# gvanhorn38/multibox

Measured on AMD Instinct MI355X. Metric: images/sec (299x299, 5-AR priors) train, higher is better.
Workload: dtype bf16; 1 GPU; full train step: Inception-ResNet-v2 + multibox heads fwd, on-device matching+loss, bwd, RMSProp+EMA; 299x299, k=5 (P=646), BATCH_SIZE=64/GPU, MAX_NUM_BBOXES=13; global_batch=64, parallelism=dp1, hip_graph=True

## Files before the change

include/mbx.h:

```cpp
#ifndef MBX_H
#define MBX_H

#include <stddef.h>
#include <stdint.h>

#ifdef __cplusplus
extern "C" {
#endif

typedef void* mbx_stream_t;

typedef enum {
  MBX_OK = 0,
  MBX_ERR_INVALID_ARG = -1,
  MBX_ERR_UNSUPPORTED = -2,
  MBX_ERR_LAUNCH = -3,
  MBX_ERR_WORKSPACE = -4
} mbx_status;

int mbx_version(void);
const char* mbx_status_string(int status);

int mbx_priors_count(int k, const int* grids, int n_grids);

// ... 96 lines not shown
                   int32_t* n_gt_counted , int32_t* status , mbx_stream_t stream);

#define MBX_COCO_ACC_MAX_R 128
#define MBX_COCO_ACC_MAX_M 4
#define MBX_COCO_ACC_MAX_ND 4194304
#define MBX_COCO_ACC_CHUNK 256
#define MBX_COCO_ACC_SORT_TILE 1024
size_t mbx_coco_accumulate_workspace(long long ND, int T, int A, int M);
int mbx_coco_accumulate(const double* dt , const int32_t* dt_rows , int I,
                        const int16_t* match , const uint8_t* ignore ,
                        const int32_t* n_gt_counted , int T, int A, const double* rec_thrs , int R,
                        const int32_t* max_dets , int M, double* precision ,
                        double* recall , void* workspace, size_t workspace_bytes, mbx_stream_t stream);

typedef enum {
  MBX_EPI_STORE = 0,
  MBX_EPI_AFFINE = 1,
  MBX_EPI_RESIDUAL = 2,
  MBX_EPI_STORE_F32 = 3
} mbx_epilogue;

typedef struct {
  int32_t n, rows_mod;
  int32_t c_begin[4];
  const void* y[4]; int32_t ld_y[4];
  const float* relu_thr[4];
  float* stats[4]; int32_t stats_ld[4];
} mbx_bn_bwd_stats;

#define MBX_GRID_BARRIER_BYTES 6400
typedef struct {
  void* barrier;
  void* a; int32_t ld_a;
  const float* beta;
  float* mean; float* rstd;
  float* moving_mean; float* moving_var;
  float* relu_thr;
  int32_t relu; float eps, decay;
  float* step_poison;
} mbx_bn_apply_desc;

#define MBX_BN_BWD_SLOTS 8
typedef struct {
  void* barrier;
  int32_t n;
  int32_t c_begin[4];
  const void* y[4]; int32_t ld_y[4];
  void* dy[4]; int32_t ld_dy[4];
  const float* mean[4]; const float* rstd[4]; const float* beta[4];
  float* dbeta[4];
  float* acc[4]; int32_t acc_ld[4];
  int32_t relu[4];
  float* step_poison;
} mbx_bn_bwd_fused;

typedef struct {
  const void* x; int64_t x_img_stride; int32_t ldx;
  int32_t N, H_in, W_in, C_in;
  const void* w; int32_t C_out, R, S;
  int32_t stride, transposed, pad_t, pad_l, H_out, W_out;
  void* y; int64_t y_img_stride; int32_t ldy;
  int32_t epilogue, relu, accumulate;
  const float* scale; const float* shift;
  const void* skip; int64_t skip_img_stride; int32_t ld_skip; float rscale;
  float* stats_partial;
  int32_t tile_config;
  const void* acc_src; int64_t acc_img_stride; int32_t ld_acc;
  int32_t* work_counter;
  int32_t max_workgroups;
  void* splitk_ws; int64_t splitk_ws_bytes;
  int32_t stats_rows_mod, stats_ld;
  const mbx_bn_bwd_stats* bn_bwd_stats;
  void* relu_bits; int32_t ld_bits;
  const mbx_bn_apply_desc* bn_apply;
  const mbx_bn_bwd_fused* bn_bwd;
} mbx_conv_desc;
#define MBX_CONV_TILE_CONFIGS 14
#define MBX_TILE_I5_BASE 32
#define MBX_TILE_I7 65
#define MBX_TILE_DIRECT3 96
#define MBX_TILE_DIRECTW 97
#define MBX_TILE_RESIDENT 98
#define MBX_TILE_PWRES 99
#define MBX_TILE_SPLITK_BASE 128
#define MBX_TILE_SPLITK_MAX 32

int mbx_conv_stats_rows(const mbx_conv_desc* desc );
int mbx_conv(const mbx_conv_desc* desc , mbx_stream_t stream);
int mbx_conv_supported(const mbx_conv_desc* desc );
int mbx_conv_pair(const mbx_conv_desc* a , const mbx_conv_desc* b , mbx_stream_t stream);
size_t mbx_conv_splitk_workspace_bytes(const mbx_conv_desc* desc );

int mbx_conv_wgrad(const mbx_conv_desc* desc , const void* dy,
                   int64_t dy_img_stride, int32_t ld_dy, float* dw, float* db, mbx_stream_t stream);

typedef struct {
  mbx_conv_desc desc;
  const void* dy; int64_t dy_img_stride; int32_t ld_dy;
  float scale;
  float* dw; float* db;
} mbx_wgrad_job;
typedef struct {
  int32_t n_layers, n_items;
  int64_t layers_off, items_off;
  int64_t queues_off, heads_off;
  double flops;
  int64_t tally_off;
} mbx_wgrad_plan_info;
#define MBX_WGRAD_DETERMINISTIC 1
#define MBX_WGRAD_SCATTER 2
size_t mbx_wgrad_plan_bytes(const mbx_wgrad_job* jobs , int n_jobs, int flags);
int mbx_wgrad_plan(const mbx_wgrad_job* jobs , int n_jobs, int flags, void* host_image, size_t bytes,
                   mbx_wgrad_plan_info* info );
int mbx_conv_wgrad_grouped(void* device_image , const mbx_wgrad_plan_info* info ,
                           mbx_stream_t stream);
int mbx_conv_wgrad_grouped_capped(void* device_image, const mbx_wgrad_plan_info* info , int max_workgroups,
                                  mbx_stream_t stream);

int mbx_conv_wgrad_scaled(const mbx_conv_desc* desc, const void* dy, int64_t dy_img_stride,
                          int32_t ld_dy, float scale, float* dw, float* db, mbx_stream_t stream);

int mbx_bn_finalize(const float* stats_partial , int rows, int C, int64_t count,
                    float eps, float decay, float* mean , float* rstd ,
                    float* moving_mean , float* moving_var ,
                    mbx_stream_t stream);
int mbx_bn_apply(const void* y, int64_t M, int C, const float* mean, const float* rstd,
                 const float* beta, int relu, void* a, int ld_a, mbx_stream_t stream);
int mbx_bn_apply_fused(const float* stats_partial, int rows, int64_t count, float eps, float decay,
                       const void* y, int64_t M, int C, const float* beta, int relu, void* a, int ld_a,
                       float* mean, float* rstd, float* moving_mean, float* moving_var,
                       mbx_stream_t stream);
int mbx_bn_apply_fused_mapped(const void* stats_fixed, int rows, int64_t count, float eps, float decay,
                              const void* y, int64_t M, int C, const float* beta, int relu, void* a, int ld_a,
                              const struct mbx_chan_map_s* a_map , float* mean, float* rstd, float* moving_mean,
                              float* moving_var, float* relu_thr, mbx_stream_t stream);
int mbx_bn_moving_update(float* moving_mean, float* moving_var, const float* batch_mean, const float* batch_var,
                         int64_t n, float decay, const float* skip_ctl, uint64_t* skipped_steps,
                         float* ema_mean, float* ema_var, float ema_decay, mbx_stream_t stream);
typedef struct mbx_chan_map_s { int32_t n; int32_t c_begin[4]; int32_t offset[4]; } mbx_chan_map;
int mbx_bn_finalize_parts(const float* const* parts , const int32_t* rows ,
                          const int32_t* Cs , int n_parts, int64_t count, float eps, float decay, float* mean,
                          float* rstd, float* moving_mean, float* moving_var, mbx_stream_t stream);
int mbx_bn_apply_mapped(const void* y, int64_t M, int C, const float* mean, const float* rstd, const float* beta,
                        int relu, void* a, int ld_a, const mbx_chan_map* a_map , mbx_stream_t stream);
int mbx_bn_apply_maxpool(const void* y, int N, int H, int W, int C, const float* mean, const float* rstd, const float* beta,
                         int relu, void* p, int64_t p_img_stride, int ld_p, int Ho, int Wo, uint8_t* argmax,
                         mbx_stream_t stream);
int mbx_bn_fold(const float* moving_mean, const float* moving_var, const float* beta, float eps,
                int C, float* scale, float* shift, mbx_stream_t stream);
int mbx_bn_bwd_rows(int64_t M, int C);
int mbx_bn_bwd_reduce(const void* da, int ld_da, const void* a, int ld_a, int relu, const void* y,
                      int64_t M, int C, const float* mean, const float* rstd, const float* beta,
                      float* partial , mbx_stream_t stream);
int mbx_bn_bwd_finalize(const float* partial, int rows, int C, int64_t M, float* dbeta ,
                        float* m12 , mbx_stream_t stream);
int mbx_bn_bwd_apply(const void* da, int ld_da, const void* a, int ld_a, int relu, const void* y,
                     int64_t M, int C, const float* mean, const float* rstd, const float* beta,
                     const float* m12, void* dy , mbx_stream_t stream);

int mbx_bn_bwd_reduce_mapped(const void* da, int ld_da, const void* a, int ld_a, int relu, const void* y, int64_t M, int C,
                             const float* mean, const float* rstd, const float* beta, float* partial,
                             const mbx_chan_map* da_map , mbx_stream_t stream);
int mbx_bn_bwd_apply_mapped(const void* da, int ld_da, const void* a, int ld_a, int relu, const void* y, int64_t M, int C,
                            const float* mean, const float* rstd, const float* beta, const float* m12, void* dy,
                            const mbx_chan_map* da_map , mbx_stream_t stream);

// ... 100 lines not shown
```

multibox_amd/build.py:

```python
from __future__ import annotations

import os
import shutil
import subprocess
import sys

HERE = os.path.dirname(os.path.abspath(__file__))
CSRC = os.path.join(HERE, "csrc")
OBJ = os.path.join(CSRC, "_obj")
LIB = os.path.join(HERE, "libmbx.so")
ARCH = "gfx950"

SOURCES = {
    "priors.cpp": ["-ffp-contract=off"],
    "loss.hip": ["-ffp-contract=off"],
    "postproc.hip": ["-ffp-contract=off"],
    "merge.hip": ["-ffp-contract=off"],
    "cocomatch.hip": ["-ffp-contract=off"],
    "cocoaccum.hip": ["-ffp-contract=off"],
    "conv.hip": ["-munsafe-fp-atomics"],
    "wgrad.hip": ["-munsafe-fp-atomics"],
    "conv5.hip": ["-mllvm", "-amdgpu-atomic-optimizer-strategy=None"],
    "conv7.hip": ["-mllvm", "-amdgpu-atomic-optimizer-strategy=None"],
    "convd.hip": [],
    "convr.hip": [],
    "nnops.hip": ["-munsafe-fp-atomics"],
    "bn.hip": ["-munsafe-fp-atomics"],
    "augment.hip": ["-ffp-contract=off"],
}
COMMON = ["-O3", "-std=c++17", "-fPIC", "--offload-arch=" + ARCH, "-Wall", "-Wno-unused-function"]
COMMON += os.environ.get("MBX_BUILD_DEFS", "").split()


def _hipcc():
    for c in (shutil.which("hipcc"), "/opt/rocm/bin/hipcc"):
        if c and os.path.exists(c):
            return c
    raise RuntimeError("hipcc not found: libmbx needs ROCm's hipcc to build")


def _newer(a, bs):
    if not os.path.exists(a):
        return True
    ta = os.path.getmtime(a)
    return any(os.path.getmtime(b) > ta for b in bs)


def build(force=False, verbose=True):
    hipcc = _hipcc()
    os.makedirs(OBJ, exist_ok=True)
    headers = [os.path.join(CSRC, f) for f in os.listdir(CSRC) if f.endswith(".h")]
    headers.append(os.path.join(os.path.dirname(HERE), "include", "mbx.h"))
    headers.append(os.path.abspath(__file__))
    objs = []
    procs = []
    for src, flags in SOURCES.items():
        s = os.path.join(CSRC, src)
        o = os.path.join(OBJ, src.rsplit(".", 1)[0] + ".o")
        objs.append(o)
        if force or _newer(o, [s] + headers):
            cmd = [hipcc] + COMMON + flags + (["-x", "hip"] if src.endswith(".hip") else []) + ["-c", s, "-o", o]
            if verbose:
                print("[mbx build]", " ".join(cmd), flush=True)
            procs.append((src, subprocess.Popen(cmd, stdout=subprocess.PIPE, stderr=subprocess.STDOUT, text=True)))
    failed = []
    for src, p in procs:
        out, _ = p.communicate()
        if p.returncode != 0:
            failed.append((src, out))
        elif verbose and out.strip():
            print(out)
    if failed:
        raise RuntimeError("hipcc failed:\n" + "\n".join("== %s ==\n%s" % f for f in failed))
    if force or _newer(LIB, objs):
        cmd = [hipcc, "-shared", "-fPIC", "--offload-arch=" + ARCH, "-o", LIB] + objs
        if verbose:
            print("[mbx build]", " ".join(cmd), flush=True)
        subprocess.check_call(cmd)
    return LIB


if __name__ == "__main__":
    build(force="--force" in sys.argv)
    print(LIB)
```

multibox_amd/csrc/conv.hip:

```cpp
#include <stdlib.h>

#include "conv_common.h"

namespace {

template <int BM, int BN, int WNW, int WMW, int EV, int MODE = 0, int NSTG = 3>
__device__ __forceinline__ void conv_igemm3_body(const ConvK& p, const int bid_, const int nblk_) {
  constexpr bool SH = MODE == 2, PW = MODE == 1;
  static_assert(WNW * WMW == 4 || WNW * WMW == 8, "four or eight waves");
  constexpr int NT = 64 * WNW * WMW, RPP = NT / 8;
  constexpr int TN = BN / WNW, TM = BM / WMW, NI = TN / 16, MI = TM / 16;
  constexpr int PI = BM / RPP, WI = BN / RPP, NL = PI + WI;
  constexpr int STAGE = (BM + BN) * 8;
  extern __shared__ __attribute__((aligned(16))) u32x4 smem[];

  const int tid = threadIdx.x, lane = tid & 63;
  const int wave = wave_id();
  const int wn = wave % WNW, wm = wave / WNW;
  int lid = xcd_remap(bid_, nblk_);
  int split = 0;
  if constexpr (EV == 5) { const int nt = p.tiles_m * p.tiles_n; split = lid / nt; lid -= split * nt; }
  const int tile_n = lid % p.tiles_n, tile_m = lid / p.tiles_n;
  const int m0 = tile_m * BM, n0 = tile_n * BN;

// ... 211 lines not shown
        a = *reinterpret_cast<const float4*>(src);
        int sl = 1;
        for (; sl + 3 < ksplit; sl += 4) {
          const float4 b0 = *reinterpret_cast<const float4*>(src + (sl + 0) * slice_stride);
          const float4 b1 = *reinterpret_cast<const float4*>(src + (sl + 1) * slice_stride);
          const float4 b2 = *reinterpret_cast<const float4*>(src + (sl + 2) * slice_stride);
          const float4 b3 = *reinterpret_cast<const float4*>(src + (sl + 3) * slice_stride);
          a.x = (((a.x + b0.x) + b1.x) + b2.x) + b3.x; a.y = (((a.y + b0.y) + b1.y) + b2.y) + b3.y;
          a.z = (((a.z + b0.z) + b1.z) + b2.z) + b3.z; a.w = (((a.w + b0.w) + b1.w) + b2.w) + b3.w;
        }
        for (; sl < ksplit; ++sl) {
          const float4 b = *reinterpret_cast<const float4*>(src + sl * slice_stride);
          a.x += b.x; a.y += b.y; a.z += b.z; a.w += b.w;
        }
      }
      const float v[4] = {a.x, a.y, a.z, a.w};
      const unsigned q2[2] = {pack2bf(v[0], v[1]), pack2bf(v[2], v[3])};
      const unsigned q[4] = {q2[0] & 0xffffu, q2[0] >> 16, q2[1] & 0xffffu, q2[1] >> 16};
#pragma unroll
      for (int j = 0; j < 4; ++j) {
        const float f = (m < M && c + j < C) ? bf2f((unsigned short)q[j]) : 0.f;
        if (4 * gq + j < 256) { red[r][4 * gq + j][0] = f; red[r][4 * gq + j][1] = f * f; }
      }
      if (m < M) {
        const int img = m / HW_out, pix = m - img * HW_out;
        unsigned short* dst = y + img * y_img_stride + (long long)pix * ldy + c;
        if (c + 3 < C) *reinterpret_cast<u32x2*>(dst) = u32x2{q2[0], q2[1]};
        else for (int j = 0; j < 4; ++j) if (c + j < C) dst[j] = (unsigned short)q[j];
      }
    }
    if (stats) {
      __syncthreads();
      if (tid < cw) {
        float x1 = 0.f, x2 = 0.f;
#pragma unroll
        for (int r = 0; r < kSplitRows; ++r) { x1 += red[r][tid][0]; x2 += red[r][tid][1]; }
        if (stats_mod) {
          unsigned long long* o = reinterpret_cast<unsigned long long*>(stats) + ((size_t)((int)blockIdx.x % stats_mod) * stats_ld + cb + tid) * 2;
          stats_add_fixed(o, x1, x2, stats_cap);
        } else {
          float* o = stats + ((size_t)blockIdx.x * stats_ld + cb + tid) * 2;
          o[0] = x1;
          o[1] = x2;
        }
      }
    }
  }
}

struct TileCfg { int BM, BN; float eff; };
const TileCfg kCfgs[] = {{128, 128, 1.00f}, {128, 64, 0.85f}, {64, 128, 0.85f}, {128, 32, 0.60f}, {64, 64, 0.70f},
                          {256, 128, 1.30f}, {128, 128, 1.10f}, {256, 64, 1.0f},
                          {128, 128, 1.10f},
                          {128, 64, 0.85f}, {64, 64, 0.70f},
                          {128, 64, 0.85f}, {256, 64, 1.0f}, {128, 128, 1.0f}};

int pick_cfg(long M, int C_out) {
  int best = 0;
  double best_t = 1e300;
  for (int i = 0; i < (int)(sizeof(kCfgs) / sizeof(kCfgs[0])); ++i) {
    if (i >= 5) continue;
    const TileCfg& c = kCfgs[i];
    const long tiles = ((M + c.BM - 1) / c.BM) * ((C_out + c.BN - 1) / c.BN);
    const long lds = 3L * (c.BM + c.BN) * 128;
    long per_cu = (160 * 1024) / lds;
    if (per_cu > 2) per_cu = 2;
    const long rounds = (tiles + 256 * per_cu - 1) / (256 * per_cu);
    const double t = (double)rounds * c.BM * c.BN / c.eff;
    if (t < best_t) { best_t = t; best = i; }
  }
  return best;
}



constexpr int kNumCfgs = MBX_CONV_TILE_CONFIGS;
static_assert(kGbCtlWords * 4 == MBX_GRID_BARRIER_BYTES && kFbSlots == MBX_BN_BWD_SLOTS, "include/mbx.h and csrc/grid_barrier.h agree");
constexpr int kI5Flag = MBX_TILE_I5_BASE;
constexpr int kI7Cfg = MBX_TILE_I7;
constexpr int kDirectCfg = MBX_TILE_DIRECT3;
constexpr int kDirectWCfg = MBX_TILE_DIRECTW;
constexpr int kResidentCfg = MBX_TILE_RESIDENT;
constexpr int kPwResCfg = MBX_TILE_PWRES;
constexpr int kSplitFlag = MBX_TILE_SPLITK_BASE;
constexpr int kSplitMax = MBX_TILE_SPLITK_MAX;
inline void splitk_geom(int nk, int S, int& ksplit, int& kps) {
  if (S > nk) S = nk;
  if (S < 1) S = 1;
  kps = (nk + S - 1) / S;
  ksplit = (nk + kps - 1) / kps;
}
int choose_cfg(long M, int C_out, int desc_cfg) {
  static const int force = mbx_env_int("MBX_FORCE_CFG", -1);
  if (force >= 0) return force;
  if (desc_cfg > 0 && desc_cfg <= kNumCfgs) return desc_cfg - 1;
  {
    const long cols = (C_out + 127) / 128, tiles8 = ((M + 127) / 128) * cols;
    if (tiles8 >= 384 && (double)C_out >= 0.6 * (double)(cols * 128)) return 8;
  }
  if (C_out >= 256) {
    const long tiles5 = ((M + 255) / 256) * ((C_out + 127) / 128);
    const long rounds5 = (tiles5 + 255) / 256;
    if (tiles5 >= 128 && (double)tiles5 / (double)(rounds5 * 256) >= 0.7) return 5;
  }
  return pick_cfg(M, C_out);
}

struct PairCapture { ConvK k; int bm, bn, wnw, wmw, nstg, ev, mode, valid; };
thread_local PairCapture g_capture;

template <int BM, int BN, int WNW, int WMW, int EV, int NSTG>
int launch_pair_inst(const ConvK& a, const ConvK& b, hipStream_t s) {
  static bool attr = false;
  const size_t lds = NSTG * (size_t)(BM + BN) * 128;
  if (!attr) {
    (void)hipFuncSetAttribute(reinterpret_cast<const void*>(conv_igemm3_pair_kernel<BM, BN, WNW, WMW, EV, 0, NSTG>),
                              hipFuncAttributeMaxDynamicSharedMemorySize, (int)lds);
    attr = true;
  }
  const int n0 = a.tiles_m * a.tiles_n, n1 = b.tiles_m * b.tiles_n;
  hipLaunchKernelGGL((conv_igemm3_pair_kernel<BM, BN, WNW, WMW, EV, 0, NSTG>), dim3(n0 + n1), dim3(64 * WNW * WMW), lds, s, a, b, n0);
  MBX_LAUNCH_CHECK();
  return MBX_OK;
}

template <int BM, int BN, int WNW, int WMW, int NSTG = 3>
int launch_igemm(ConvK& k, hipStream_t s) {
  k.tiles_m = (k.M + BM - 1) / BM;
  k.tiles_n = (k.C_out + BN - 1) / BN;
  k.stats_cap = stats_cap_for(k.tiles_m);
  if (k.dry == 2) {
    g_capture.k = k; g_capture.bm = BM; g_capture.bn = BN; g_capture.wnw = WNW; g_capture.wmw = WMW; g_capture.nstg = NSTG;
    g_capture.ev = k.epi == MBX_EPI_STORE_F32 ? 5 : k.epi == MBX_EPI_RESIDUAL ? 4 : k.epi == MBX_EPI_AFFINE ? 3
                   : k.bw_n ? 6 : k.stats ? 1 : (k.accumulate || k.skip || k.bits) ? 2 : 0;
    g_capture.mode = k.shift ? 2 : k.pw ? 1 : 0;
    g_capture.valid = 1;
    return MBX_OK;
  }
  {
    const size_t lds = NSTG * (size_t)(BM + BN) * 128;
    const int ev = k.epi == MBX_EPI_STORE_F32 ? 5 : k.epi == MBX_EPI_RESIDUAL ? 4 : k.epi == MBX_EPI_AFFINE ? 3
                   : k.bw_n ? 6 : k.stats ? 1 : (k.accumulate || k.skip || k.bits) ? 2 : 0;
    static bool attr_set3[7] = {false, false, false, false, false, false, false};
#define MBX_LAUNCH_EV(EV)                                                                                     \
    case EV:                                                                                                  \
      if (!attr_set3[EV]) {                                                                                   \
        (void)hipFuncSetAttribute(reinterpret_cast<const void*>(conv_igemm3_kernel<BM, BN, WNW, WMW, EV, 0, NSTG>), \
                                  hipFuncAttributeMaxDynamicSharedMemorySize, (int)lds);                      \
        (void)hipFuncSetAttribute(reinterpret_cast<const void*>(conv_igemm3_kernel<BM, BN, WNW, WMW, EV, 1, NSTG>), \
                                  hipFuncAttributeMaxDynamicSharedMemorySize, (int)lds);                      \
        attr_set3[EV] = true;                                                                                 \
      }                                                                                                       \
      if (k.pw)                                                                                               \
        hipLaunchKernelGGL((conv_igemm3_kernel<BM, BN, WNW, WMW, EV, 1, NSTG>), dim3(k.tiles_m * k.tiles_n * (EV == 5 ? k.ksplit : 1)), \
                           dim3(64 * WNW * WMW), lds, s, k);                                                  \
      else                                                                                                    \
        hipLaunchKernelGGL((conv_igemm3_kernel<BM, BN, WNW, WMW, EV, 0, NSTG>), dim3(k.tiles_m * k.tiles_n * (EV == 5 ? k.ksplit : 1)), \
                           dim3(64 * WNW * WMW), lds, s, k);                                                  \
      break;
    static bool attr_sh[2] = {false, false};
#define MBX_LAUNCH_SH(EV, SLOT)                                                                               \
    do {                                                                                                      \
      if (!attr_sh[SLOT]) {                                                                                   \
        (void)hipFuncSetAttribute(reinterpret_cast<const void*>(conv_igemm3_kernel<BM, BN, WNW, WMW, EV, 2, NSTG>), \
                                  hipFuncAttributeMaxDynamicSharedMemorySize, (int)lds);                      \
        attr_sh[SLOT] = true;                                                                                 \
// ... 176 lines not shown
      return MBX_ERR_INVALID_ARG;
    for (int i = 0; i < b->n; ++i) {
      if (!b->y[i] || !b->relu_thr[i] || !b->stats[i] || (reinterpret_cast<uintptr_t>(b->y[i]) & 15) || b->ld_y[i] % 8 || b->c_begin[i] % 32 ||
          b->c_begin[i] >= d->C_out || (i && b->c_begin[i] <= b->c_begin[i - 1]) || b->stats_ld[i] <= 0)
        return MBX_ERR_INVALID_ARG;
      k.bw_cb[i] = b->c_begin[i]; k.bw_ldy[i] = b->ld_y[i]; k.bw_sld[i] = b->stats_ld[i];
      k.bw_y[i] = reinterpret_cast<const unsigned short*>(b->y[i]); k.bw_thr[i] = b->relu_thr[i]; k.bw_stats[i] = b->stats[i];
    }
    k.bw_n = b->n; k.bw_mod = b->rows_mod;
  }
  if (d->accumulate && d->acc_src) {
    if (d->ld_acc % 8 || (reinterpret_cast<uintptr_t>(d->acc_src) & 15) || (long long)d->N * d->acc_img_stride >= (1LL << 31))
      return MBX_ERR_INVALID_ARG;
    k.acc_src = reinterpret_cast<const unsigned short*>(d->acc_src); k.acc_img_stride = (int)d->acc_img_stride; k.ld_acc = d->ld_acc;
  } else {
    k.acc_src = reinterpret_cast<const unsigned short*>(d->y); k.acc_img_stride = (int)d->y_img_stride; k.ld_acc = d->ldy;
  }
  {
    const long long last_pix = (long long)k.HW_out - 1, span = ((d->C_out + 7) / 8) * 8;
    const long long yb = 2 * ((long long)(d->N - 1) * d->y_img_stride + last_pix * d->ldy + span);
    const long long sb = d->skip ? 2 * ((long long)(d->N - 1) * d->skip_img_stride + last_pix * d->ld_skip + span) : 0;
    const long long ab = 2 * ((long long)(d->N - 1) * k.acc_img_stride + last_pix * k.ld_acc + span);
    if (!f32 && (yb >= (1LL << 31) || sb >= (1LL << 31) || ab >= (1LL << 31))) return MBX_ERR_UNSUPPORTED;
    k.y_bytes = (unsigned)yb; k.skip_bytes = (unsigned)sb; k.acc_bytes = (unsigned)ab;
  }
  set_magic((unsigned)k.HW_out, k.mg_hw, k.sh_hw);
  set_magic((unsigned)k.W_out, k.mg_w, k.sh_w);
  k.pw = (d->R == 1 && d->S == 1 && d->pad_t == 0 && d->pad_l == 0 && d->stride == 1) ? 1 : 0;
  k.skip_taps = 0; k.parity = 0;
  k.work_counter = d->work_counter;
  k.max_wg = d->max_workgroups;
  k.dry = dry;
  k.ksplit = 1; k.kps = 1 << 30; k.y_split_stride = 0;
#ifdef MBX_I5_STAMPS
  {
    static const unsigned long long sp = getenv("MBX_I5_STAMP_PTR") ? strtoull(getenv("MBX_I5_STAMP_PTR"), nullptr, 10) : 0ull;
    k.stamps = reinterpret_cast<unsigned long long*>(sp);
    k.dbg = mbx_env_int("MBX_I5_DBG", 0);
    k.stagger = mbx_env_int("MBX_STAGGER", 0);
  }
#endif
  for (int c = 0; c < 4; ++c) { k.cls_m0[c] = 0; k.cls_hw[c] = 1; k.cls_w[c] = 1; }
  static const bool notap = mbx_env_char("MBX_NO_TAP_SKIP") == '1';
  if (k.shift && d->C_in % 64 == 0 && !notap) {
    int m0 = 0;
    for (int c = 0; c < 4; ++c) {
      const int hc = (d->H_out - (c >> 1) + 1) / 2, wc = (d->W_out - (c & 1) + 1) / 2;
      k.cls_m0[c] = m0;
      k.cls_hw[c] = hc * wc > 0 ? hc * wc : 1;
      k.cls_w[c] = wc > 0 ? wc : 1;
      m0 += d->N * hc * wc;
    }
    k.skip_taps = k.parity = 1;
  }
  if (k.bits && k.shift) return MBX_ERR_UNSUPPORTED;
  hipStream_t s = mbx_s(stream);
  if (d->tile_config > kSplitFlag) {
    const int S = d->tile_config - kSplitFlag;
    if (S < 2 || S > kSplitMax || d->transposed || d->bn_bwd_stats || d->relu_bits || d->epilogue != MBX_EPI_STORE || d->accumulate || d->skip || d->rscale != 0.f)
      return MBX_ERR_UNSUPPORTED;
    const int ldp = ((d->C_out + 7) / 8) * 8;
    int ksplit, kps;
    splitk_geom((k.Ktot + 63) >> 6, S, ksplit, kps);
    const long long slice = (long long)k.M * ldp;
    if (!d->splitk_ws || (reinterpret_cast<uintptr_t>(d->splitk_ws) & 15) || d->splitk_ws_bytes < (int64_t)(4 * slice * ksplit) ||
        slice * ksplit >= (1LL << 31))
      return MBX_ERR_WORKSPACE;
    ConvK g = k;
    g.epi = MBX_EPI_STORE_F32; g.stats = nullptr; g.relu = 0;
    g.y = d->splitk_ws; g.ldy = ldp; g.y_img_stride = k.HW_out * ldp;
    g.ksplit = ksplit; g.kps = kps; g.y_split_stride = slice;
    st = launch_igemm<128, 64, 2, 2>(g, s);
    if (st != MBX_OK || dry) return st;
    hipLaunchKernelGGL(splitk_reduce_kernel, dim3((k.M + kSplitRows - 1) / kSplitRows), dim3(256), 0, s, reinterpret_cast<const float*>(d->splitk_ws),
                       ksplit, slice, k.M, k.C_out, ldp, reinterpret_cast<unsigned short*>(k.y), k.HW_out,
                       (long long)k.y_img_stride, k.ldy, k.stats, k.stats_mod, k.stats_ld, stats_cap_for((k.M + kSplitRows - 1) / kSplitRows));
    MBX_LAUNCH_CHECK();
    return MBX_OK;
  }
  if (d->tile_config == kDirectCfg) return mbx_launch_direct3(k, d->N, d->H_out, s);
  if (d->tile_config == kDirectWCfg) return mbx_launch_directw(k, d->N, d->H_out, s);
  if (d->tile_config == kResidentCfg) return mbx_launch_resident(k, d->N, d->H_out, s);
  if (d->tile_config == kPwResCfg) return mbx_launch_pwres(k, s);
  if (d->tile_config == kI7Cfg) return mbx_launch_igemm7(k, s);
  if (d->tile_config > kI5Flag) return mbx_launch_igemm5(k, d->tile_config - kI5Flag - 1, s);
  switch (choose_cfg(k.M, k.C_out, d->tile_config)) {
    case 0: return launch_igemm<128, 128, 2, 2>(k, s);
    case 1: return launch_igemm<128, 64, 2, 2>(k, s);
    case 2: return launch_igemm<64, 128, 2, 2>(k, s);
    case 3: return launch_igemm<128, 32, 1, 4>(k, s);
    case 5: return launch_igemm<256, 128, 2, 4>(k, s);
    case 6: return launch_igemm<128, 128, 2, 4>(k, s);
    case 7: return launch_igemm<256, 64, 1, 8>(k, s);
    case 8: return launch_igemm<128, 128, 2, 4, 2>(k, s);
    case 9: return launch_igemm<128, 64, 2, 2, 2>(k, s);
    case 10: return launch_igemm<64, 64, 2, 2, 2>(k, s);
    case 11: return launch_igemm<128, 64, 2, 4, 2>(k, s);
    case 12: return launch_igemm<256, 64, 1, 8, 2>(k, s);
    case 13: return launch_igemm<128, 128, 2, 2, 2>(k, s);
    default: return launch_igemm<64, 64, 2, 2>(k, s);
  }
}
```

multibox_amd/csrc/conv_common.h:

```cpp
#pragma once
#include <type_traits>
#include "common.h"
#include "grid_barrier.h"

namespace mbx {

struct ConvK {
  const unsigned short* x; int x_img_stride, ldx, H_in, W_in, C_in;
  const unsigned short* w; int C_out, R, S, Ktot;
  unsigned x_bytes, w_bytes;
  unsigned y_bytes, skip_bytes, acc_bytes;
  int mul, shift, pad_t, pad_l, W_out, HW_out, M;
  void* y; int y_img_stride, ldy;
  int epi, relu, accumulate;
  const float* scale; const float* shiftv;
  const unsigned short* skip; int skip_img_stride, ld_skip; float rscale;
  const unsigned short* acc_src; int acc_img_stride, ld_acc;
  unsigned char* bits; int bits_ld; unsigned bits_bytes;
  float* stats;
  float stats_cap;
  int stats_mod, stats_ld;
  int bw_n, bw_mod;
  int bw_cb[4], bw_ldy[4], bw_sld[4];
  const unsigned short* bw_y[4];
  const float* bw_thr[4];
  float* bw_stats[4];
  FusedApply fa;
  FusedBwd fb;
  int tiles_m, tiles_n;
  unsigned mg_hw, sh_hw, mg_w, sh_w;
  int pw;
  int cls_m0[4], cls_hw[4], cls_w[4];
  int skip_taps;
  int parity;
  int* work_counter;
  int max_wg;
  int dry;
  int ksplit, kps; long long y_split_stride;
#ifdef MBX_I5_STAMPS
  unsigned long long* stamps;
  int dbg;
  int stagger;
#endif
};

}

int mbx_launch_igemm5(mbx::ConvK& k, int index, hipStream_t s);
extern const int mbx_i5_tiles[][2];
extern const int mbx_i5_num_tiles;
int mbx_launch_igemm7(mbx::ConvK& k, hipStream_t s);
int mbx_launch_direct3(mbx::ConvK& k, int N, int H_out, hipStream_t s);
int mbx_direct3_grid(int N, int H_out, int W_out);
int mbx_launch_directw(mbx::ConvK& k, int N, int H_out, hipStream_t s);
int mbx_directw_grid(int N, int H_out, int W_out);
int mbx_launch_resident(mbx::ConvK& k, int N, int H_out, hipStream_t s);
int mbx_resident_rows(int N);
int mbx_launch_pwres(mbx::ConvK& k, hipStream_t s);

namespace {

using mbx::ConvK;
using mbx::FusedApply;
using mbx::FusedBwd;

typedef __attribute__((ext_vector_type(8))) __bf16 bf16x8;
typedef __attribute__((ext_vector_type(4))) float f32x4;
typedef __attribute__((ext_vector_type(4))) short s16x4;
typedef __attribute__((ext_vector_type(4))) unsigned int u32x4;
typedef __attribute__((ext_vector_type(2))) unsigned int u32x2;

__device__ __forceinline__ float bf2f(unsigned short h) { return __uint_as_float(((unsigned)h) << 16); }
__device__ __forceinline__ unsigned short f2bf(float f) { return __builtin_bit_cast(unsigned short, (__bf16)f); }
typedef float f32x4u __attribute__((ext_vector_type(4), aligned(4)));
__device__ __forceinline__ unsigned pack2bf(float lo, float hi) {
  typedef float pk_f32x2 __attribute__((ext_vector_type(2)));
  typedef __bf16 pk_bf16x2 __attribute__((ext_vector_type(2)));
  return __builtin_bit_cast(unsigned, __builtin_convertvector(pk_f32x2{lo, hi}, pk_bf16x2));
}
__device__ __forceinline__ float bf_lo(unsigned w) { return __uint_as_float(w << 16); }
__device__ __forceinline__ float bf_hi(unsigned w) { return __uint_as_float(w & 0xffff0000u); }
__device__ __forceinline__ unsigned gather4_rows(unsigned b) {
  typedef unsigned g4_u32x2 __attribute__((ext_vector_type(2)));
  const g4_u32x2 r = __builtin_amdgcn_permlane16_swap(b, b, false, false);
  const unsigned t = r.x | (r.y << 8);
  const g4_u32x2 q = __builtin_amdgcn_permlane32_swap(t, t, false, false);
  return q.x | (q.y << 16);
}
__device__ __forceinline__ float relu_f(float x) {
  float r;
  asm("v_max_f32 %0, 0, %1" : "=v"(r) : "v"(x));
  return r;
}

constexpr int kThreads = 256;

inline int conv_cus() { const int n = mbx_cu_count(); return n ? n : 256; }

inline bool store_or_affine_only(const ConvK& k) {
  return (k.epi == MBX_EPI_STORE || k.epi == MBX_EPI_AFFINE) && !k.accumulate && !k.skip && !k.bits && k.rscale == 0.f && !k.bw_n &&
         !(k.epi == MBX_EPI_AFFINE && k.stats);
}

template <typename Q, typename F>
inline int launch_by_ev(const ConvK& k, const Q& q, int grid, int threads, int lds, hipStream_t s, F kern) {
  static bool attr[3] = {false, false, false};
  const int ev = k.epi == MBX_EPI_AFFINE ? 2 : k.stats ? 1 : 0;
  void (*const fn)(const ConvK, const Q) = ev == 2 ? kern(std::integral_constant<int, 3>())
                                           : ev   ? kern(std::integral_constant<int, 1>()) : kern(std::integral_constant<int, 0>());
  if (!attr[ev]) {
    (void)hipFuncSetAttribute(reinterpret_cast<const void*>(fn), hipFuncAttributeMaxDynamicSharedMemorySize, lds);
    attr[ev] = true;
  }
  hipLaunchKernelGGL(fn, dim3(grid), dim3(threads), lds, s, k, q);
  MBX_LAUNCH_CHECK();
  return MBX_OK;
}

inline void set_magic(unsigned d, unsigned& mg, unsigned& sh) {
  unsigned l = 0;
  while ((1ull << l) < d) ++l;
  sh = 31 + l;
  mg = (unsigned)((1ull << sh) / d + 1);
}

inline int check_desc(const mbx_conv_desc* d) {
  if (!d || !d->x || !d->N || d->N < 0) return MBX_ERR_INVALID_ARG;
  if (d->C_in <= 0 || d->C_in % 8 || d->ldx % 8 || d->ldx < d->C_in) return MBX_ERR_INVALID_ARG;
  if (d->R <= 0 || d->S <= 0 || d->C_out <= 0 || d->H_out <= 0 || d->W_out <= 0) return MBX_ERR_INVALID_ARG;
  if (d->stride != 1 && d->stride != 2) return MBX_ERR_UNSUPPORTED;
  if ((reinterpret_cast<uintptr_t>(d->x) & 15)) return MBX_ERR_INVALID_ARG;
  const long long xe = (long long)d->N * d->x_img_stride;
  if (xe >= (1LL << 30) || (long long)d->N * d->H_out * d->W_out >= (1LL << 31)) return MBX_ERR_UNSUPPORTED;
  return MBX_OK;
}

__device__ __forceinline__ float row_sum16(float v) {
  asm volatile("s_nop 1\n\t"
               "v_add_f32_dpp %0, %0, %0 row_ror:8 row_mask:0xf bank_mask:0xf\n\t"
               "s_nop 1\n\t"
               "v_add_f32_dpp %0, %0, %0 row_ror:4 row_mask:0xf bank_mask:0xf\n\t"
// ... 364 lines not shown
```

multibox_amd/ops.py:

```python
from __future__ import annotations

import ctypes as C
import os

import torch

from . import _lib

EPI_STORE, EPI_AFFINE, EPI_RESIDUAL, EPI_STORE_F32 = 0, 1, 2, 3


class ConvDesc(C.Structure):
    _fields_ = [
        ("x", C.c_void_p), ("x_img_stride", C.c_int64), ("ldx", C.c_int32),
        ("N", C.c_int32), ("H_in", C.c_int32), ("W_in", C.c_int32), ("C_in", C.c_int32),
        ("w", C.c_void_p), ("C_out", C.c_int32), ("R", C.c_int32), ("S", C.c_int32),
        ("stride", C.c_int32), ("transposed", C.c_int32), ("pad_t", C.c_int32), ("pad_l", C.c_int32),
        ("H_out", C.c_int32), ("W_out", C.c_int32),
        ("y", C.c_void_p), ("y_img_stride", C.c_int64), ("ldy", C.c_int32),
        ("epilogue", C.c_int32), ("relu", C.c_int32), ("accumulate", C.c_int32),
        ("scale", C.c_void_p), ("shift", C.c_void_p),
        ("skip", C.c_void_p), ("skip_img_stride", C.c_int64), ("ld_skip", C.c_int32), ("rscale", C.c_float),
        ("stats_partial", C.c_void_p),
        ("tile_config", C.c_int32),
# ... 161 lines not shown
I7_COUNTERS = 32
SPLITK_FLAG = 128
DIRECT3_TILE_CONFIG = 96


def direct3_applies(desc: ConvDesc, min_pixels=300000):
    if os.environ.get("MBX_DIRECT3", "1") == "0":
        return False
    if desc.R != 3 or desc.S != 3 or desc.epilogue not in (EPI_STORE, EPI_AFFINE) or desc.accumulate or desc.skip \
            or desc.rscale != 0.0 or (desc.epilogue == EPI_AFFINE and desc.stats_partial) or desc.bn_bwd_stats:
        return False
    if desc.stride == 2 and not desc.transposed and desc.C_in == 8 and desc.C_out <= 32 and desc.C_out % 8 == 0:
        pass
    elif desc.stride != 1 or desc.C_in not in (32, 64) or desc.C_out > 64 or desc.C_out % 8 or (desc.C_in == 64 and desc.C_out > 48):
        return False
    if -(-desc.W_out // 32) * 32 > 1.15 * desc.W_out:
        return False
    return desc.N * desc.H_out * desc.W_out >= int(os.environ.get("MBX_DIRECT3_MIN_PIXELS", min_pixels))


DIRECTW_TILE_CONFIG = 97


def directw_applies(desc: ConvDesc, min_pixels=60000):
    if os.environ.get("MBX_DIRECTW", "1") == "0":
        return False
    if desc.R != 3 or desc.S != 3 or desc.stride != 1 or desc.epilogue not in (EPI_STORE, EPI_AFFINE) or desc.accumulate or desc.skip \
            or desc.rscale != 0.0 or (desc.epilogue == EPI_AFFINE and desc.stats_partial) or desc.bn_bwd_stats:
        return False
    if desc.C_in not in (32, 48, 64) or desc.C_out > 64 or desc.C_out % 8 or (desc.C_in == 64 and desc.C_out > 48):
        return False
    if not (8 <= desc.W_out <= 64) or desc.W_in > desc.W_out + 2:
        return False
    return desc.N * desc.H_out * desc.W_out >= int(os.environ.get("MBX_DIRECTW_MIN_PIXELS", min_pixels))


RESIDENT_TILE_CONFIG = 98


def resident_applies(desc: ConvDesc, min_images=32):
    if os.environ.get("MBX_RESIDENT", "1") == "0":
        return False
    if desc.R * desc.S not in (3, 7) or min(desc.R, desc.S) != 1 or desc.stride != 1 or desc.epilogue not in (EPI_STORE, EPI_AFFINE) \
            or desc.accumulate or desc.skip or desc.rscale != 0.0 or (desc.epilogue == EPI_AFFINE and desc.stats_partial) \
            or desc.bn_bwd_stats or desc.relu_bits:
        return False
    if desc.H_in != desc.H_out or desc.W_in != desc.W_out or not (64 <= desc.H_out * desc.W_out <= 289):
        return False
    if desc.N < int(os.environ.get("MBX_RESIDENT_MIN_IMAGES", min_images)):
        return False
    if not desc.x or not desc.w or not desc.y:
        hw = desc.H_out * desc.W_out
        if desc.C_out % 8:
            return False
        if desc.R * desc.S == 3:
            return hw == 64 and desc.C_in in (192, 224, 256)
        return 65 <= hw <= 289 and desc.C_in in (128, 160, 192)
    keep = desc.tile_config
    desc.tile_config = RESIDENT_TILE_CONFIG
    ok = _lib.lib().mbx_conv_supported(C.byref(desc)) == 0
    desc.tile_config = keep
    return ok


PWRES_DEFAULT = "2"
PWRES_TILE_CONFIG = 99


def pwres_applies(desc: ConvDesc, min_pixels=4096):
    mode = os.environ.get("MBX_PWRES", PWRES_DEFAULT)
    if mode == "0":
        return False
    if desc.R != 1 or desc.S != 1 or desc.stride != 1 or desc.pad_t or desc.pad_l or desc.stats_partial or desc.bn_bwd_stats:
        return False
    if desc.C_in not in (96, 128, 320, 384, 448) or desc.C_out < 256 or desc.C_out % 8:
        return False
    res = desc.epilogue == EPI_RESIDUAL
    accm = desc.epilogue == EPI_STORE and desc.relu_bits and not desc.skip
    if not (res or accm) or (mode == "2" and not accm):
        return False
    return desc.N * desc.H_out * desc.W_out >= int(os.environ.get("MBX_PWRES_MIN_PIXELS", min_pixels))


def launch_rule(desc: ConvDesc, pair=False):
    if direct3_applies(desc):
        return DIRECT3_TILE_CONFIG, "direct 3x3"
    if directw_applies(desc) and not pair:
        return DIRECTW_TILE_CONFIG, "direct 3x3 (whole-width)"
    if pwres_applies(desc):
        return PWRES_TILE_CONFIG, "pixel-resident 1x1"
    if resident_applies(desc):
        return RESIDENT_TILE_CONFIG, "resident image"
    return None


def splitk_slices(desc: ConvDesc, n_cus=256):
    if os.environ.get("MBX_SPLITK", "1") == "0" or desc.transposed or desc.epilogue != EPI_STORE or desc.accumulate or desc.skip:
        return 0
    ktot = desc.R * desc.S * desc.C_in
    M = desc.N * desc.H_out * desc.W_out
    tiles = ((M + 127) // 128) * ((desc.C_out + 63) // 64)
    if ktot < 8192 or tiles > 96:
        return 0
    s = int(os.environ.get("MBX_SPLITK_SLICES", "0")) or max(2, min(16, (2 * n_cus) // tiles))
    return min(s, 32)
_TUNED = {}
TUNE_STATS = {"hits": 0, "remeasured": 0, "rejected": 0}
_TUNE_FILE = os.path.join(os.path.dirname(os.path.abspath(__file__)), "tune_cache.json")


def _load_tune_cache():
    if os.environ.get("MBX_TUNE_CACHE", "1") != "0" and os.path.exists(_TUNE_FILE):
        try:
            import json
            with open(_TUNE_FILE) as f:
                _TUNED.update({k: int(v) for k, v in json.load(f).items()})
        except (OSError, ValueError):
            pass


def save_tune_cache(path=None):
    import json
    with open(path or _TUNE_FILE, "w") as f:
        json.dump(dict(sorted(_TUNED.items())), f, indent=0)


_load_tune_cache()


def autotune(desc: ConvDesc, key, candidates=None, iters=10):
    key = repr(key)
    if key in _TUNED:
        desc.tile_config = _TUNED[key]
        if _lib.lib().mbx_conv_supported(C.byref(desc)) == 0:
            TUNE_STATS["hits"] += 1
            return desc.tile_config
        del _TUNED[key]
        TUNE_STATS["rejected"] += 1
    TUNE_STATS["remeasured"] += 1
    if candidates is None:
        candidates = (0, 2, 4, 5, 6, 9, 10, 12, 13, 14)
        if os.environ.get("MBX_AUTOTUNE_SET") == "all":
            candidates = tuple(range(0, N_TILE_CONFIGS + 1))
    l = _lib.lib()
    best, best_t = 0, float("inf")
    s = _stream()
    iters = int(os.environ.get("MBX_TUNE_ITERS", iters))
    for cfg in candidates:
        desc.tile_config = cfg
        if l.mbx_conv(C.byref(desc), s) != 0:
            continue
        e0, e1 = torch.cuda.Event(enable_timing=True), torch.cuda.Event(enable_timing=True)
        e0.record()
        for _ in range(iters):
            l.mbx_conv(C.byref(desc), s)
        e1.record()
        e1.synchronize()
        t = e0.elapsed_time(e1)
        if t < best_t * 0.97 or (cfg == 0 and t < best_t):
            best, best_t = cfg, t
    desc.tile_config = best
    _TUNED[key] = best
    return best


def autotune_wgrad(desc: ConvDesc, dy: View, scale, dw, db, key, candidates=(0, 2, 3, 4, 7, 8, 9, 10), iters=10):
    key = repr(key)
    if key in _TUNED:
        desc.tile_config = _TUNED[key]
        return desc.tile_config
    l = _lib.lib()
# ... 57 lines not shown
```

Measured before the change: 4336 images/sec.

## Add filter-resident streaming kernel for small pointwise convolutions

Adds a new 1x1 convolution kernel that loads the whole filter into LDS once per workgroup, then streams 16-pixel blocks through waves. Each wave double-buffers its activation loads and runs MFMA against the resident filter. It is routed to only for two specific (C_in, C_out) shapes with a plain store epilogue, and skipped for paired launches. The aim is to cut repeated filter reloads and tile overhead of the general implicit-GEMM path for narrow-output 1x1 convs. The cost is another specialised kernel whose LDS use and per-wave streaming may limit occupancy.

```diff
diff --git a/include/mbx.h b/include/mbx.h
--- a/include/mbx.h
+++ b/include/mbx.h
@@ -202,6 +202,7 @@
 #define MBX_TILE_DIRECTW 97
 #define MBX_TILE_RESIDENT 98
 #define MBX_TILE_PWRES 99
+#define MBX_TILE_PWSTREAM 100
 #define MBX_TILE_SPLITK_BASE 128
 #define MBX_TILE_SPLITK_MAX 32
 
diff --git a/multibox_amd/build.py b/multibox_amd/build.py
--- a/multibox_amd/build.py
+++ b/multibox_amd/build.py
@@ -24,6 +24,7 @@
     "conv7.hip": ["-mllvm", "-amdgpu-atomic-optimizer-strategy=None"],
     "convd.hip": [],
     "convr.hip": [],
+    "convs.hip": [],
     "nnops.hip": ["-munsafe-fp-atomics"],
     "bn.hip": ["-munsafe-fp-atomics"],
     "augment.hip": ["-ffp-contract=off"],
diff --git a/multibox_amd/csrc/conv.hip b/multibox_amd/csrc/conv.hip
--- a/multibox_amd/csrc/conv.hip
+++ b/multibox_amd/csrc/conv.hip
@@ -317,6 +317,7 @@
 constexpr int kDirectWCfg = MBX_TILE_DIRECTW;
 constexpr int kResidentCfg = MBX_TILE_RESIDENT;
 constexpr int kPwResCfg = MBX_TILE_PWRES;
+constexpr int kPwStreamCfg = MBX_TILE_PWSTREAM;
 constexpr int kSplitFlag = MBX_TILE_SPLITK_BASE;
 constexpr int kSplitMax = MBX_TILE_SPLITK_MAX;
 inline void splitk_geom(int nk, int S, int& ksplit, int& kps) {
@@ -659,6 +660,7 @@
   if (d->tile_config == kDirectWCfg) return mbx_launch_directw(k, d->N, d->H_out, s);
   if (d->tile_config == kResidentCfg) return mbx_launch_resident(k, d->N, d->H_out, s);
   if (d->tile_config == kPwResCfg) return mbx_launch_pwres(k, s);
+  if (d->tile_config == kPwStreamCfg) return mbx_launch_pwstream(k, s);
   if (d->tile_config == kI7Cfg) return mbx_launch_igemm7(k, s);
   if (d->tile_config > kI5Flag) return mbx_launch_igemm5(k, d->tile_config - kI5Flag - 1, s);
   switch (choose_cfg(k.M, k.C_out, d->tile_config)) {
diff --git a/multibox_amd/csrc/conv_common.h b/multibox_amd/csrc/conv_common.h
--- a/multibox_amd/csrc/conv_common.h
+++ b/multibox_amd/csrc/conv_common.h
@@ -57,6 +57,7 @@
 int mbx_launch_resident(mbx::ConvK& k, int N, int H_out, hipStream_t s);
 int mbx_resident_rows(int N);
 int mbx_launch_pwres(mbx::ConvK& k, hipStream_t s);
+int mbx_launch_pwstream(mbx::ConvK& k, hipStream_t s);
 
 namespace {
 
diff --git a/multibox_amd/csrc/convs.hip b/multibox_amd/csrc/convs.hip
--- /dev/null
+++ b/multibox_amd/csrc/convs.hip
@@ -0,0 +1,154 @@
+#include "direct_epilogue.h"
+
+namespace {
+
+constexpr int kSThreads = 512;
+constexpr int kSWaves = kSThreads / 64;
+
+struct StrK {
+  int nblk;
+};
+
+template <int C8>
+__device__ __forceinline__ int skey(int r) {
+  return (C8 % 16 == 0) ? 2 * (r & 7) : (C8 % 16 == 8) ? 2 * ((r >> 1) & 3) : 2 * ((r >> 2) & 1);
+}
+template <int C8> constexpr int sjx() { return (C8 % 16 == 0) ? 3 : (C8 % 16 == 8) ? 1 : 0; }
+template <int C8>
+__device__ __forceinline__ int sencb(int row, int fch) {
+  const int k = skey<C8>(row);
+  return 16 * (row * C8 + (fch ^ (k & 3)) + 4 * (k >> 2));
+}
+typedef const __attribute__((address_space(3))) u32x4* slds_u32x4_cptr;
+__device__ __forceinline__ int lds_addr_s(const void* p) { return (int)(unsigned)(size_t)((const __attribute__((address_space(3))) char*)p); }
+template <int C8>
+__device__ __forceinline__ bf16x8 sread(int Eb, int a, int j) {
+  const unsigned addr = (unsigned)((Eb ^ (64 * (j & sjx<C8>()))) + 64 * (j & ~sjx<C8>()) + a * (16 * C8 * 16));
+  return __builtin_bit_cast(bf16x8, *(slds_u32x4_cptr)(size_t)addr);
+}
+
+template <int KC, int NB>
+struct StrG {
+  static constexpr int C8 = 4 * KC;
+  static constexpr int ROWS = 16 * NB;
+  static constexpr int FCH = (ROWS * C8 + 511) / 512 * 512;
+  static constexpr int LDS_BYTES = FCH * 16;
+};
+
+template <int KC, int NB>
+__global__ void __launch_bounds__(kSThreads)
+conv_pwres_kernel_stream(const ConvK p, const StrK q) {
+  using G = StrG<KC, NB>;
+  constexpr int C8 = G::C8, ROWS = G::ROWS;
+  constexpr int D = KC * NB < 6 ? KC * NB : 6;
+  extern __shared__ __attribute__((aligned(16))) u32x4 smem[];
+  u32x4* const filt = smem;
+  const int lane = threadIdx.x & 63;
+  const int wave = wave_id();
+  const int frow = lane & 15, fch = lane >> 4;
+  const __amdgpu_buffer_rsrc_t xr = make_rsrc(p.x, p.x_bytes);
+  const __amdgpu_buffer_rsrc_t wr = make_rsrc(p.w, p.w_bytes);
+  const __amdgpu_buffer_rsrc_t yr = make_rsrc(p.y, p.y_bytes);
+  const int first = xcd_remap((int)blockIdx.x, (int)gridDim.x);
+  const int stride = (int)gridDim.x * kSWaves;
+  const int c8 = p.C_in >> 3;
+
+  auto load_x = [&](const int b, bf16x8 (&x)[KC]) {
+    const int m = 16 * b + frow;
+    const bool pv = m < p.M;
+    const int img = (int)fast_div((unsigned)(pv ? m : 0), p.mg_hw, p.sh_hw);
+    const int xo = (img * p.x_img_stride + (m - img * p.HW_out) * p.ldx + fch * 8) * 2;
+#pragma unroll
+    for (int j = 0; j < KC; ++j)
+      x[j] = __builtin_bit_cast(bf16x8, buf_load16(xr, (pv && 4 * j + fch < c8) ? (unsigned)(xo + j * 64) : kOOB));
+  };
+
+  int b = first * kSWaves + wave;
+  bf16x8 x0[KC], x1[KC];
+#pragma unroll
+  for (int i0 = 0; i0 < G::FCH / 64; i0 += kSWaves) {
+    const int i = i0 + wave;
+    const int ci = i * 64 + lane;
+    const int row = ci / C8, cs = ci - row * C8;
+    const int c = cs ^ skey<C8>(row);
+    const int ch = dperm<ROWS>(row >> 4, row & 15);
+    glds16(wr, filt + i * 64, (row < ROWS && ch < p.C_out && c < c8) ? (ch * p.Ktot + c * 8) * 2 : (int)kOOB);
+  }
+  __builtin_amdgcn_sched_barrier(0);
+  load_x(b, x0);
+  __builtin_amdgcn_sched_barrier(0);
+  wait_vmcnt<KC>();
+  lds_readback_wait(lds_readback_issue(filt + lane));
+  raw_barrier();
+
+  const int EA = sencb<C8>(frow, fch) + lds_addr_s(smem);
+  const DirAffine<NB> af{};
+  const float rs = p.rscale != 0.f ? p.rscale : 1.f;
+
+  auto step = [&](const int blk, const bf16x8 (&x)[KC], bf16x8 (&xn)[KC]) {
+    const int mlane = 16 * blk + frow;
+    load_x(blk + stride, xn);
+    __builtin_amdgcn_sched_barrier(0);
+    f32x4 acc[NB][1];
+#pragma unroll
+    for (int a = 0; a < NB; ++a) acc[a][0] = f32x4{0.f, 0.f, 0.f, 0.f};
+    constexpr int NS = NB * KC;
+    bf16x8 wf[D];
+#pragma unroll
+    for (int s = 0; s < D; ++s) wf[s] = sread<C8>(EA, s / KC, s % KC);
+    __builtin_amdgcn_sched_barrier(0);
+#pragma unroll
+    for (int s = 0; s < NS; ++s) {
+      acc[s / KC][0] = __builtin_amdgcn_mfma_f32_16x16x32_bf16(wf[s % D], x[s % KC], acc[s / KC][0], 0, 0, 0);
+      if (s + D < NS) wf[s % D] = sread<C8>(EA, (s + D) / KC, (s + D) % KC);
+      __builtin_amdgcn_sched_barrier(0);
+    }
+    const bool pv = mlane < p.M;
+    const int img = (int)fast_div((unsigned)(pv ? mlane : 0), p.mg_hw, p.sh_hw);
+    float s1[NB][4], s2[NB][4];
+#pragma unroll
+    for (int a = 0; a < NB; ++a) acc[a][0] *= rs;
+    direct_store_pixel<0>(p, yr, acc, 0, pv, img * p.y_img_stride + (mlane - img * p.HW_out) * p.ldy, 0, p.C_out, fch, af, s1, s2);
+    __builtin_amdgcn_sched_barrier(0);
+  };
+
+  while (b < q.nblk) {
+    step(b, x0, x1);
+    b += stride;
+    if (b >= q.nblk) break;
+    step(b, x1, x0);
+    b += stride;
+  }
+}
+
+template <int KC, int NB>
+int launch_stream(const ConvK& k, hipStream_t s) {
+  using G = StrG<KC, NB>;
+  static_assert(G::LDS_BYTES <= 96 * 1024, "LDS");
+  StrK q;
+  q.nblk = (k.M + 15) / 16;
+  const int need = (q.nblk + kSWaves - 1) / kSWaves;
+  int grid = need < conv_cus() ? need : conv_cus();
+  if (k.max_wg > 0 && grid > k.max_wg) grid = k.max_wg;
+  if (k.dry) return MBX_OK;
+  static bool attr = false;
+  if (!attr) {
+    (void)hipFuncSetAttribute(reinterpret_cast<const void*>(conv_pwres_kernel_stream<KC, NB>), hipFuncAttributeMaxDynamicSharedMemorySize, G::LDS_BYTES);
+    attr = true;
+  }
+  hipLaunchKernelGGL((conv_pwres_kernel_stream<KC, NB>), dim3(grid), dim3(kSThreads), G::LDS_BYTES, s, k, q);
+  MBX_LAUNCH_CHECK();
+  return MBX_OK;
+}
+
+}
+
+int mbx_launch_pwstream(ConvK& k, hipStream_t s) {
+  if (!k.pw || k.shift || k.mul != 1 || k.bw_n || k.C_out % 8 || k.accumulate || k.stats || k.fa.bar || k.fb.bar) return MBX_ERR_UNSUPPORTED;
+  if (k.epi != MBX_EPI_STORE || k.skip || k.bits) return MBX_ERR_UNSUPPORTED;
+  const int KC = (k.C_in + 31) / 32, NB = (k.C_out + 15) / 16;
+  if ((long long)NB * 16 * KC * 64 > 96 * 1024) return MBX_ERR_UNSUPPORTED;
+  if (KC == 10 && NB == 8) return launch_stream<10, 8>(k, s);
+  if (KC == 3 && NB == 4) return launch_stream<3, 4>(k, s);
+  return MBX_ERR_UNSUPPORTED;
+}
diff --git a/multibox_amd/ops.py b/multibox_amd/ops.py
--- a/multibox_amd/ops.py
+++ b/multibox_amd/ops.py
@@ -267,11 +267,40 @@
     return desc.N * desc.H_out * desc.W_out >= int(os.environ.get("MBX_PWRES_MIN_PIXELS", min_pixels))
 
 
+PWSTREAM_TILE_CONFIG = 100
+PWSTREAM_BUILT = ((320, 128), (80, 64))
+PWSTREAM_SHAPES = ((320, 128), (80, 64))
+
+
+def pwstream_applies(desc: ConvDesc, min_pixels=4096):
+    mode = os.environ.get("MBX_PWSTREAM", "1")
+    if mode == "0":
+        return False
+    if desc.R != 1 or desc.S != 1 or desc.stride != 1 or desc.pad_t or desc.pad_l or desc.accumulate or desc.stats_partial \
+            or desc.bn_bwd_stats or desc.bn_apply or desc.bn_bwd or desc.epilogue != EPI_STORE or desc.skip or desc.relu_bits:
+        return False
+    shapes = PWSTREAM_SHAPES if mode == "1" else PWSTREAM_BUILT if mode == "all" else \
+        tuple(tuple(int(v) for v in s.split("x")) for s in mode.split(",") if s)
+    if (desc.C_in, desc.C_out) not in shapes:
+        return False
+    if desc.N * desc.H_out * desc.W_out < int(os.environ.get("MBX_PWSTREAM_MIN_PIXELS", min_pixels)):
+        return False
+    if not desc.x or not desc.w or not desc.y:
+        return True
+    keep = desc.tile_config
+    desc.tile_config = PWSTREAM_TILE_CONFIG
+    ok = _lib.lib().mbx_conv_supported(C.byref(desc)) == 0
+    desc.tile_config = keep
+    return ok
+
+
 def launch_rule(desc: ConvDesc, pair=False):
     if direct3_applies(desc):
         return DIRECT3_TILE_CONFIG, "direct 3x3"
     if directw_applies(desc) and not pair:
         return DIRECTW_TILE_CONFIG, "direct 3x3 (whole-width)"
+    if pwstream_applies(desc) and not pair:
+        return PWSTREAM_TILE_CONFIG, "filter-resident streaming 1x1"
     if pwres_applies(desc):
         return PWRES_TILE_CONFIG, "pixel-resident 1x1"
     if resident_applies(desc):
```

New measurement: 4344 images/sec (median of 6 runs). Within noise of the previous version (+0.2%).
